# zynthbox/libzl

Hardware: AMD Instinct MI355X
Metric: voice-samples/sec at 1024 voices x 256-frame blocks; % HBM roofline (higher is better)
Workload: dtype f32

## Files before the change

libzl_amd/build.py:

```python
from __future__ import annotations

import os
import shutil
import subprocess
import sys

ROOT = os.path.dirname(os.path.dirname(os.path.abspath(__file__)))
CSRC = os.path.join(ROOT, "libzl_amd", "csrc")
LIBDIR = os.path.join(ROOT, "libzl_amd", "lib")
LIB = os.path.join(LIBDIR, "libzlhip.so")

HIP_SOURCES = ["zl_kernels.hip", "zl_stretch.hip", "zl_overview.hip", "zl_onset.hip", "zl_tempo.hip", "zl_pitch.hip", "zl_loudness.hip", "zl_loop.hip", "zl_key.hip", "zl_xfade.hip", "zl_decode.hip", "zl_resample.hip", "zl_engine.cpp", "zl_clip_calls.cpp", "zl_libzl.cpp", "zl_group.cpp"]
HEADERS = ["zl_types.h", "zl_arena.h", "zl_plan.h", "zl_order.h", "zl_pair.h", "zl_launch.h", "zl_render.h", "zl_kernels.h", "zl_host.h", "zl_sched.h", "zl_handoff.h", "zl_stretch.h", "zl_overview.h", "zl_onset.h", "zl_tempo.h", "zl_pitch.h", "zl_loudness.h", "zl_loop.h", "zl_key.h", "zl_xfade.h", "zl_decode.h", "zl_resample.h", "zl_group.h", "zl_member.h", "zl_owned.h", "zl_engine_impl.h",
           os.path.join("..", "..", "include", "zlhip.h"), os.path.join("..", "..", "include", "libzl_hotpath.h")]


def _hipcc() -> str:
    for cand in (os.environ.get("HIPCC"), shutil.which("hipcc"), "/opt/rocm/bin/hipcc"):
        if cand and os.path.exists(cand):
            return cand
    raise RuntimeError("hipcc not found (needed to build libzlhip.so for gfx950)")


def _stale(target: str, deps: list[str]) -> bool:
# ... 144 lines not shown
    if ref is None:
        return None
    odir = os.path.join(ROOT, "oracle")
    target = REF_LIB_CONTRACTED if contracted else REF_LIB
    voice = os.path.join(ref, "lib", "SamplerSynthVoice.cpp")
    driver = os.path.join(odir, "ref_driver.cpp")
    shim = os.path.join(odir, "ref_shim")
    deps = [voice, driver, os.path.join(odir, "zl_oracle.c"), os.path.join(odir, "zl_oracle.h"), os.path.abspath(__file__)]
    deps += [os.path.join(d, f) for d, _, fs in os.walk(shim) for f in fs]
    deps += [os.path.join(ref, "lib", f) for f in os.listdir(os.path.join(ref, "lib")) if f.endswith(".h")]
    if not force and not _stale(target, deps):
        return target
    os.makedirs(os.path.dirname(target), exist_ok=True)
    fp = ["-O2", "-mfma", "-ffp-contract=fast"] if contracted else ["-O2", "-ffp-contract=off", "-fno-fast-math"]
    cobj = os.path.join(os.path.dirname(target), "zl_oracle_fma.o" if contracted else "zl_oracle.o")
    cmds = [["gcc", "-std=c11", "-O2", "-ffp-contract=off", "-fno-fast-math", "-fPIC", "-c", os.path.join(odir, "zl_oracle.c"), "-o", cobj],
            ["g++", "-std=c++17"] + fp + ["-fPIC", "-shared", "-Wall", "-Wl,-Bsymbolic", "-I", shim, "-I", odir, "-I", os.path.join(ref, "lib"),
                                          "-o", target, voice, driver, cobj, "-lm", "-lpthread"]]
    for cmd in cmds:
        res = subprocess.run(cmd, capture_output=True, text=True)
        if res.returncode != 0:
            sys.stderr.write(res.stdout + res.stderr)
            raise RuntimeError("building the reference voice failed")
    return target


_ZLHIP_H = os.path.join(_INC, "zlhip.h")
_NO_CONTRACT = ["-ffp-contract=off", "-fno-fast-math"]


def _build_harness(name: str, source: str, headers: list, flags: list, force: bool = False) -> str:
    hdir = os.path.join(ROOT, "tests", "cpu_harness")
    target = os.path.join(hdir, "_build", f"lib{name}.so")
    src = os.path.join(hdir, source)
    if force or _stale(target, [src] + [os.path.join(CSRC, h) for h in headers]):
        os.makedirs(os.path.dirname(target), exist_ok=True)
        cmd = ["g++", "-std=c++17", "-O2"] + flags + ["-fPIC", "-shared", "-Wl,-Bsymbolic", "-I", CSRC, "-I", os.path.join(ROOT, "include"), "-o", target, src]
        res = subprocess.run(cmd, capture_output=True, text=True)
        if res.returncode != 0:
            sys.stderr.write(res.stdout + res.stderr)
            raise RuntimeError(f"building the CPU test harness {source} failed")
    return target


def build_cpu_harness(force: bool = False) -> str:
    target = _build_harness("zl_plan_host", "plan_host.cpp", ["zl_types.h", "zl_plan.h", "zl_render.h", "zl_host.h", _ZLHIP_H], _NO_CONTRACT, force)
    _build_harness("zl_sched_host", "sched_host.cpp", ["zl_sched.h", _ZLHIP_H], _NO_CONTRACT + ["-Wall"], force)
    _build_harness("zl_stretch_host", "stretch_host.cpp", ["zl_stretch.h", "zl_types.h"], _NO_CONTRACT + ["-Wall", "-pthread"], force)
    return target


def build_order_harness(force: bool = False) -> str:
    return _build_harness("zl_order_host", "order_host.cpp", ["zl_types.h", "zl_plan.h", "zl_order.h", "zl_host.h", _ZLHIP_H], _NO_CONTRACT + ["-Wall", "-Wno-unused-function"], force)


def build_order_summary_harness(force: bool = False) -> str:
    return _build_harness("zl_order_summary_host", "order_summary_host.cpp", ["zl_types.h", "zl_order.h"], ["-Wall", "-Wno-unused-function"], force)


def build_ongrid_harness(force: bool = False) -> str:
    return _build_harness("zl_ongrid_host", "ongrid_host.cpp", ["zl_types.h", "zl_render.h"], _NO_CONTRACT + ["-Wall", "-Wno-unused-function"], force)


def build_ongrid_pk_harness(force: bool = False) -> str:
    return _build_harness("zl_ongrid_pk_host", "ongrid_pk_host.cpp", ["zl_types.h", "zl_render.h"], _NO_CONTRACT + ["-Wall", "-Wno-unused-function"], force)


def build_pair_harness(force: bool = False) -> str:
    return _build_harness("zl_pair_host", "pair_host.cpp", ["zl_pair.h"], ["-Wall"], force)


def build_pair_wrap_harness(force: bool = False) -> str:
    plan_host = os.path.join("..", "..", "tests", "cpu_harness", "plan_host.cpp")
    return _build_harness("zl_pair_wrap_host", "pair_wrap_host.cpp", ["zl_types.h", "zl_plan.h", "zl_render.h", "zl_host.h", _ZLHIP_H, plan_host],
                          _NO_CONTRACT + ["-Wall", "-Wno-unused-function"], force)


def build_pair_scalar_harness(force: bool = False) -> str:
    plan_host = os.path.join("..", "..", "tests", "cpu_harness", "plan_host.cpp")
    return _build_harness("zl_pair_scalar_host", "pair_scalar_host.cpp", ["zl_types.h", "zl_plan.h", "zl_render.h", "zl_order.h", "zl_pair.h", "zl_host.h", _ZLHIP_H, plan_host],
                          _NO_CONTRACT + ["-Wall", "-Wno-unused-function"], force)


def build_group_harness(force: bool = False) -> str:
    return _build_harness("zl_group_host", "group_host.cpp", ["zl_types.h", "zl_plan.h", "zl_host.h", "zl_group.h", _ZLHIP_H], _NO_CONTRACT + ["-Wall", "-Wno-unused-function"], force)


def build_overview_harness(force: bool = False) -> str:
    return _build_harness("zl_overview_host", "overview_host.cpp", ["zl_types.h", "zl_overview.h"], ["-Wall"], force)


def build_onset_harness(force: bool = False) -> str:
    return _build_harness("zl_onset_host", "onset_host.cpp", ["zl_types.h", "zl_stretch.h", "zl_overview.h", "zl_onset.h"], _NO_CONTRACT + ["-Wall", "-pthread"], force)


def build_tempo_harness(force: bool = False) -> str:
    return _build_harness("zl_tempo_host", "tempo_host.cpp", ["zl_types.h", "zl_stretch.h", "zl_overview.h", "zl_onset.h", "zl_tempo.h"], _NO_CONTRACT + ["-Wall", "-pthread"], force)


def build_pitch_harness(force: bool = False) -> str:
    return _build_harness("zl_pitch_host", "pitch_host.cpp", ["zl_types.h", "zl_stretch.h", "zl_overview.h", "zl_onset.h", "zl_pitch.h"], _NO_CONTRACT + ["-Wall", "-pthread"], force)


def build_loudness_harness(force: bool = False) -> str:
    return _build_harness("zl_loudness_host", "loudness_host.cpp", ["zl_types.h", "zl_overview.h", "zl_loudness.h"], _NO_CONTRACT + ["-Wall", "-pthread"], force)


def build_loop_harness(force: bool = False) -> str:
    return _build_harness("zl_loop_host", "loop_host.cpp", ["zl_types.h", "zl_stretch.h", "zl_overview.h", "zl_onset.h", "zl_pitch.h", "zl_loop.h"], _NO_CONTRACT + ["-Wall", "-pthread"], force)


def build_key_harness(force: bool = False) -> str:
    return _build_harness("zl_key_host", "key_host.cpp", ["zl_types.h", "zl_stretch.h", "zl_overview.h", "zl_onset.h", "zl_pitch.h", "zl_key.h"], _NO_CONTRACT + ["-Wall", "-pthread"], force)


def build_xfade_harness(force: bool = False) -> str:
    return _build_harness("zl_xfade_host", "xfade_host.cpp", ["zl_types.h", "zl_stretch.h", "zl_overview.h", "zl_onset.h", "zl_pitch.h", "zl_xfade.h", _ZLHIP_H], _NO_CONTRACT + ["-Wall"], force)


def build_decode_harness(force: bool = False) -> str:
    return _build_harness("zl_decode_host", "decode_host.cpp", ["zl_types.h", "zl_decode.h"], _NO_CONTRACT + ["-Wall"], force)


def build_resample_harness(force: bool = False) -> str:
    return _build_harness("zl_resample_host", "resample_host.cpp", ["zl_types.h", "zl_resample.h"], _NO_CONTRACT + ["-Wall"], force)


def build_arena_harness(force: bool = False) -> str:
    return _build_harness("zl_arena_host", "arena_host.cpp", ["zl_types.h", "zl_stretch.h", "zl_arena.h"], ["-Wall"], force)


def build_launch_harness(force: bool = False) -> str:
    return _build_harness("zl_launch_host", "launch_host.cpp", ["zl_types.h", "zl_order.h", "zl_pair.h", "zl_launch.h"], ["-Wall", "-Wno-unused-function"], force)


if __name__ == "__main__":
    force = "--force" in sys.argv
    print(build_engine(force=force, verbose=True))
    print(build_oracle(force=force))
```

libzl_amd/csrc/zl_engine.cpp:

```cpp
#include <hip/hip_runtime.h>
#include <sys/resource.h>

#include <algorithm>
#include <atomic>
#include <cmath>
#include <cstdio>
#include <cstdlib>
#include <chrono>
#include <cstring>
#include <mutex>
#include <string>
#include <utility>
#include <vector>

#include "../../include/zlhip.h"
#include "zl_engine_impl.h"
#include "zl_kernels.h"
#include "zl_member.h"
#include "zl_order.h"
#include "zl_pair.h"
#include "zl_plan.h"
#include "zl_render.h"

#define ZL_RT_SPLIT_MIN_VOICES 32
// ... 713 lines not shown
                              const zlhip_passthrough_params *fan_params, float *fan_out_dev, void *stream)
{
    return render_batch_impl(e, nblocks, nframes, clocks, bus_out_dev, 0, 0, fan_params, fan_out_dev, stream);
}

static int render_batch_impl(zlhip_engine *e, int32_t nblocks, int32_t nframes, const zlhip_clock *clocks, float *bus_out_dev, long long bus_stride,
                             long long ch_stride, const zlhip_passthrough_params *fan_params, float *fan_out_dev, void *stream)
{
    if (!e || !clocks || ((fan_params == nullptr) != (fan_out_dev == nullptr))) return ZLHIP_ERR_INVALID;
    if (nblocks < 1 || nblocks > e->cfg.max_batch_blocks) return fail(e, ZLHIP_ERR_CAPACITY, "nblocks exceeds max_batch_blocks");
    if (nframes < 1 || nframes > e->cfg.max_frames)
        return fail(e, ZLHIP_ERR_INVALID, "nframes must be in [1, max_frames]");
    if (e->failed) return fail(e, ZLHIP_ERR_STATE, "engine failed (the resident kernel stopped answering in the middle of a cycle): destroy it");
    ZL_HIP(e, hipSetDevice(e->device));
    { int r_ = rt_stop(e); if (r_ != ZLHIP_OK) return r_; }
    hipStream_t s = stream ? (hipStream_t)stream : e->stream;

    static const bool callStamps = std::getenv("ZL_CALL_STAMPS") != nullptr;
    const auto tEnter = std::chrono::steady_clock::now();
    zlhip_engine::CallSlot &c = e->slots[e->callIndex & 1u];
    if (c.inflight) {
        ZL_HIP(e, hipEventSynchronize(c.done));
        c.inflight = false;
        int hrc = harvest_slot(e, c);
        if (hrc != ZLHIP_OK) return hrc;
    }
    c.doneGen ^= 1u; c.done = c.doneEv[c.doneGen];
    const auto tSlot = std::chrono::steady_clock::now();
    bool regular = true;
    for (int k = 0; k < nblocks; ++k) {
        ZlHostControl::fill_clock(c.clocks.h[k], clocks[k], nframes);
        if (c.clocks.h[k].usecs_per_frame >= (1ull << 21) || c.clocks.h[k].usecs_per_frame != c.clocks.h[0].usecs_per_frame
            || (k > 0 && c.clocks.h[k].current_usecs < c.clocks.h[k - 1].current_usecs)) regular = false;
    }

    ZlBatch A; std::memset(&A, 0, sizeof A);
    A.V = e->V; A.B = e->cfg.num_buses; A.VPB = e->cfg.voices_per_bus; A.N = nframes; A.Ktot = nblocks;
    A.G = pick_group(e, nblocks, nframes);
    A.groups = (A.VPB + A.G - 1) / A.G;
    A.NB = zl_k2_narrow_buses(nblocks, A.groups, A.VPB, A.B, nframes);
    A.clocks_regular = regular ? 1 : 0;
    A.mode = e->cfg.mode;
    A.ongrid = zl_ongrid_switch();
    A.staged = (e->staged && !e->trace && nframes % 64 == 0) ? 1 : 0;
    A.sounds = e->dSounds; A.clips = e->dClips; A.arena = e->arena;
    A.voices = e->dVoices; A.reports = c.dReports; A.pass_cache = e->dPassCache;
    A.bus = bus_out_dev ? bus_out_dev : e->dBus; A.stats = c.dStats;
    A.bus_stride = bus_stride; A.ch_stride = ch_stride;
    A.trace = 0; A.pos_trace = nullptr;
    int32_t *traceBase = nullptr;
    if (e->trace) {
        const size_t need = (size_t)nblocks * e->V * nframes;
        if (need > e->traceInts) {
            ZlQuiesce quiet(e);
            e->traceInts = 0;
            ZL_HIP(e, e->dTrace.alloc(need));
            e->traceInts = need;
        }
        ZL_HIP(e, hipMemsetAsync(e->dTrace, 0xff, need * sizeof(int32_t), s));
        A.trace = 1; traceBase = e->dTrace; e->traceK = nblocks; e->traceN = nframes;
#ifdef ZL_STAMPS
        A.trace = 0;
#endif
    }

    static const int windowMulEnv = [] { const char *v = std::getenv("ZL_WINDOW_MUL"); const int m = v ? std::atoi(v) : 0; return m < 0 ? 0 : (m > 64 ? 64 : m); }();
    bool cheap = nframes >= 256;
    for (const ZlHostVoice &hv : e->hc.voices) if (hv.isPlaying && !hv.cheapPlan) { cheap = false; break; }
    int windowMul = windowMulEnv;
    if (windowMul == 0) windowMul = cheap ? 4 : 1;
    const size_t mul = e->maxGroups > 1 ? 1 : (size_t)windowMul;
    std::vector<std::pair<int, int>> &wins = e->wins;
    zlhip_engine::CallSlot &prev = e->slots[(e->callIndex + 1u) & 1u];
    const bool behindPrev = prev.inflight && hipEventQuery(prev.done) == hipErrorNotReady;
    const char *fw = std::getenv("ZL_FIRST_WINDOW_FRAMES");
    const int fwFrames = fw ? std::atoi(fw) : 0;
    zl_plan_windows(nblocks, nframes, e->windowBlocks, e->windowFrames, e->windowCap, mul, e->ps[1].hdr != nullptr, behindPrev, fw ? &fwFrames : nullptr, wins);
    const int nwin = (int)wins.size();
    const int phaseMode = [] { const char *v = std::getenv("ZL_K2_PHASE_ORDER"); return v ? std::atoi(v) : 1; }();
    const double loopFrames = phaseMode == 1 ? e->hc.phase_order_loop_frames() : INFINITY;
    const int pairMode = [] { const char *v = std::getenv("ZL_K2_PAIR"); return v ? std::atoi(v) : 1; }();
    const int stageNorun = [] { const char *v = std::getenv("ZL_K2_STAGE_NORUN"); return v ? (std::atoi(v) != 0 ? 1 : 0) : 1; }();
    const int pairScalar = [] { const char *v = std::getenv("ZL_K2_PAIR_SCALAR"); return v ? (std::atoi(v) != 0 ? 1 : 0) : 1; }();
    const bool direct = e->bnc.sink.on && e->bnc.sink.hostDev && A.groups == 1;
    const ZlK2Switches &k2sw = zl_k2_switches();
    auto k2Launch = [&](int K, bool orderTable) {
        ZlK2In in;
        in.mode = A.mode; in.N = nframes; in.K = K; in.B = A.B; in.groups = A.groups; in.NB = A.NB;
        in.staged = A.staged; in.trace = A.trace; in.ongrid = A.ongrid; in.fan = fan_out_dev != nullptr; in.host_out = direct;
        in.order_mode = phaseMode; in.call_blocks = nblocks; in.bounce = e->bnc.sink.on; in.order_table = orderTable; in.loop_frames = loopFrames;
        in.pair_mode = pairMode; in.cheap = cheap;
        return zl_k2_launch(in, k2sw);
    };
    {
        size_t need = 0;
        for (const auto &wk : wins) { const ZlK2Launch L = k2Launch(wk.second, true); if (L.order) need = std::max(need, zl_order_ints((int)L.gz, wk.second, e->V)); }
        if (need > e->ps[0].orderInts || (e->ps[1].hdr != nullptr && need > e->ps[1].orderInts)) {
            ZlQuiesce quiet(e);
            for (auto &q : e->ps) {
                if (need <= q.orderInts || q.hdr == nullptr) continue;
                q.orderInts = 0;
                ZL_HIP(e, q.order.alloc(need));
                q.orderInts = need;
            }
        }
    }
    const bool overlap = e->ps[1].hdr != nullptr && (nwin > 1 || behindPrev || e->bnc.active);
    hipStream_t ps = overlap ? e->planStream : s;
    if (e->lastPlanStream && e->lastPlanStream != ps && e->lastPlanEvent) ZL_HIP(e, hipStreamWaitEvent(ps, e->lastPlanEvent, 0));
    if (nblocks == 1) { A.inline_clock = 1; A.clock0 = c.clocks.h[0]; A.fuse_assemble = 1; }
    if (fan_out_dev) {
        for (int b = 0; b < A.B; ++b) c.pass.h[b] = pass_params(fan_params[b]);
        ZL_HIP(e, hipMemcpyAsync(c.dPass, c.pass.h, (size_t)A.B * sizeof(ZlPassParams), hipMemcpyHostToDevice, ps));
        A.pass = c.dPass; A.fan = fan_out_dev;
    }
    int rc = upload_ops(e, c, A);
    if (rc != ZLHIP_OK) return rc;
    if (e->profiling) {
        if (behindPrev && prev.profiled && e->lastRenderStream == s) c.beginEv = prev.done;
        else { ZL_HIP(e, hipEventRecord(c.evBegin, s)); c.beginEv = c.evBegin; }
    }
    e->lastRenderStream = s;
    const unsigned phase = e->ps[1].hdr != nullptr ? e->setPhase : 0u;
    const bool fusedReports = k2Launch(wins[0].second, false).scans_levels && !(e->bnc.sink.on && !direct);
    c.fusedDone = fusedReports;
    for (int w = 0; w < nwin; ++w) {
        zlhip_engine::PlanSet &q = e->ps[(phase + (unsigned)w) & 1u];
        ZlBatch Aw = A;
        Aw.k0 = wins[(size_t)w].first;
        Aw.K = wins[(size_t)w].second;
        Aw.clocks = c.clocks.d + Aw.k0;
        Aw.levels = e->dLevels + (size_t)Aw.k0 * A.B;
        Aw.pos_trace = traceBase ? traceBase + (size_t)Aw.k0 * e->V * nframes : nullptr;
        Aw.vconst = q.vconst; Aw.runs = q.runs; Aw.tsegs = q.tsegs; Aw.plan_hdr = q.hdr; Aw.plan_seg0 = q.seg0; Aw.plan_seg1 = q.seg1;
        Aw.ctl_P = q.ctlP; Aw.ctl_env = q.ctlEnv; Aw.partials = q.partials;
        Aw.ctl_next = q.ctlNext; Aw.sim_const = q.simConst;
        Aw.ctl_slots = e->ctlSlotsOverride >= 0 ? std::min<int>(e->ctlSlotsOverride, (int)(e->ctlPoolFrames / (size_t)nframes)) : (int)std::min<size_t>(e->ctlPoolFrames / (size_t)nframes, 0x7fffffff);
        Aw.ctl_base = q.ctlBase;
        q.ctlBase += (unsigned long long)Aw.K * (unsigned long long)e->V + 1ull;
        const ZlK2Launch L = k2Launch(Aw.K, q.order != nullptr);
        Aw.order = L.order ? q.order : nullptr;
        if (zl_pair_scalar_window(pairScalar, L.kernel == ZL_K2_PAIR_PHASE_RENDER, L.order, q.pairTab != nullptr && Aw.K <= e->windowCap, A.VPB)) {
            Aw.ongrid |= ZL_ONGRID_SCALAR;
            zl_batch_set_pair_tab(Aw, q.pairTab);
        }
        if (w > 0) { Aw.n_op_ranges = 0; Aw.ops = nullptr; Aw.op_ranges = nullptr; Aw.n_clip_edits = 0; Aw.clip_edits = nullptr; }
        if (ps != s && q.used) ZL_HIP(e, hipStreamWaitEvent(ps, q.renderedEv, 0));
        ZL_KERNEL(e, zl_launch_apply_ops(Aw, ps));
        ZL_KERNEL(e, zl_launch_plan(Aw, e->forceSlow, ps));
        if (ps != s && e->asmStream && !Aw.fuse_assemble) {
            ZL_HIP(e, hipEventRecord(q.k1done, ps));
            ZL_HIP(e, hipStreamWaitEvent(e->asmStream, q.k1done, 0));
            ZL_KERNEL(e, zl_launch_assemble(Aw, e->asmStream));
            if (L.order) ZL_KERNEL(e, zl_launch_order(Aw, q.order, (int)L.gz, stageNorun, e->asmStream));
            ZL_HIP(e, hipEventRecord(q.planned, e->asmStream));
            ZL_HIP(e, hipStreamWaitEvent(s, q.planned, 0));
        } else {
            if (!Aw.fuse_assemble) ZL_KERNEL(e, zl_launch_assemble(Aw, ps));
            if (L.order) ZL_KERNEL(e, zl_launch_order(Aw, q.order, (int)L.gz, stageNorun, ps));
            if (ps != s) {
                ZL_HIP(e, hipEventRecord(q.planned, ps));
                ZL_HIP(e, hipStreamWaitEvent(s, q.planned, 0));
            }
        }
        const bool k3 = !L.scans_levels;
        if (direct) { Aw.host_out = e->bnc.sink.hostDev; Aw.host_fmt = e->bnc.sink.pcm ? 1 : 0; Aw.host_total = (long long)e->bnc.sink.totalFrames; Aw.host_k0 = 0; }
        const bool closes = fusedReports && w == nwin - 1;
        if (fusedReports) { Aw.fused_reports = 1; Aw.rep_gain = e->dGain; Aw.rep_host = c.reports.d; Aw.rep_host_gain = c.gain.d; Aw.rep_host_stats = c.stats.d; }
        Aw.pair = (L.kernel == ZL_K2_PAIR_RENDER || L.kernel == ZL_K2_PAIR_PHASE_RENDER) ? 1 : 0;
        hipEvent_t k2stop = closes ? c.done : (e->profiling ? c.evK2[2 * (size_t)w + 1] : nullptr);
        ZL_KERNEL(e, zl_launch_render(Aw, L, s, e->profiling ? c.evK2[2 * (size_t)w] : nullptr, k2stop));
        if (k3) ZL_KERNEL(e, zl_launch_finalize(Aw, nullptr, s));
        if (e->bnc.sink.on && !direct) { int d_ = bounce_deliver_window(e, A.bus, 0, Aw.B, Aw.k0, Aw.K, nblocks, nframes, s); if (d_ != ZLHIP_OK) return d_; }
        if (e->ps[1].hdr != nullptr) {
            if (k2stop && !k3) q.renderedEv = k2stop;
            else { ZL_HIP(e, hipEventRecord(q.rendered, s)); q.renderedEv = q.rendered; }
            q.used = true;
        }
    }
    c.windows = nwin;
    if (ps != s) { ZL_HIP(e, hipEventRecord(e->evPlanTail, ps)); e->lastPlanEvent = e->evPlanTail; }
    else e->lastPlanEvent = c.done;
    e->lastPlanStream = ps;
    if (e->ps[1].hdr != nullptr) e->setPhase = (phase + (unsigned)nwin) & 1u;
    if (fusedReports) {
        if (e->profiling) c.profiled = true;
    } else {
        ZL_KERNEL(e, zl_launch_reports(c.dReports, e->V, e->dGain, c.reports.d, c.gain.d, c.dStats, c.stats.d, s, e->profiling ? nullptr : c.done));
        if (e->profiling) { ZL_HIP(e, hipEventRecord(c.evEnd, s)); c.profiled = true; ZL_HIP(e, hipEventRecord(c.done, s)); }
    }
    c.inflight = true;
    if (s != e->stream) e->joins[0] = c.done;
    e->latest = &c;
    e->callIndex += 1;
    e->lastK = nblocks; e->lastN = nframes; e->lastBus = bus_stride ? nullptr : A.bus; e->lastWindows = nwin;
    e->outstanding = true; e->reportsFresh = true;
    if (callStamps) {
        const auto tEnd = std::chrono::steady_clock::now();
        auto us = [](auto a, auto b) { return std::chrono::duration<double, std::micro>(b - a).count(); };
        std::fprintf(stderr, "zlhip_render_batch #%u: slot wait %.0f us, commands %.0f us, %d window(s)\n", e->callIndex - 1, us(tEnter, tSlot), us(tSlot, tEnd), nwin);
    }
    return ZLHIP_OK;
}

int zlhip_host_alloc(size_t bytes, void **out)
{
    if (!out || bytes == 0) return ZLHIP_ERR_INVALID;
    *out = nullptr;
    return hipHostMalloc(out, bytes) == hipSuccess ? ZLHIP_OK : ZLHIP_ERR_CAPACITY;
}

void zlhip_host_free(void *p) { if (p) { ZlQuiesce quiet(nullptr); (void)hipHostFree(p); } }

static int bounce_body(zlhip_engine *e, int64_t nblocks, int32_t nframes, const zlhip_clock *clocks, void *host_out, bool pcm, int64_t chunk)
{
    constexpr int NBUF = zlhip_engine::Bounce::NBUF;
    zlhip_engine::Bounce &q = e->bnc;
    const size_t total = (size_t)nblocks * (size_t)nframes;
    static const bool stamps = std::getenv("ZL_BOUNCE_STAMPS") != nullptr;
    auto now_us = [] { return std::chrono::duration<double, std::micro>(std::chrono::steady_clock::now().time_since_epoch()).count(); };
    const double t00 = stamps ? now_us() : 0.0;
    const int directMode = [] { const char *v = std::getenv("ZL_BOUNCE_DIRECT"); return v ? std::atoi(v) : 2; }();
    void *hostDev = nullptr;
    if (directMode >= (pcm ? 1 : 2)) {
        if (hipHostGetDevicePointer(&hostDev, host_out, 0) != hipSuccess) { hostDev = nullptr; (void)hipGetLastError(); }
    }
// ... 638 lines not shown
```

libzl_amd/csrc/zl_kernels.hip:

```cpp
#include <hip/hip_runtime.h>
#include <hip/hip_ext.h>
#include <algorithm>
#include <cstddef>
#include "zl_types.h"
#include "zl_plan.h"
#include "zl_render.h"
#include "zl_order.h"
#include "zl_pair.h"
#include "zl_kernels.h"

static __device__ __forceinline__ void zl_apply_clip_edit(const ZlBatch &A, const ZlClipEdit *ed, int lane)
{
    static_assert(offsetof(ZlClip, slice_pos) == ZL_CLIP_HEAD_BYTES && sizeof(ZlClip) % 16 == 0 && offsetof(ZlClipEdit, c) % 16 == 0, "clip record layout");
    const int clip = ed->clip;
    const int n16 = ed->full ? (int)(sizeof(ZlClip) / 16) : ZL_CLIP_HEAD_BYTES / 16;
    const uint4 *src = reinterpret_cast<const uint4 *>(&ed->c);
    uint4 *dst = reinterpret_cast<uint4 *>(const_cast<ZlClip *>(A.clips) + clip);
    for (int w = lane; w < n16; w += 64) dst[w] = src[w];
}

__global__ void zl_k0_apply_ops(const ZlBatch A)
{
    const int opGroups = (A.n_op_ranges + 63) / 64;
    if ((int)blockIdx.x >= opGroups) {
// ... 1470 lines not shown

template <uint32_t MODE, int BPW, bool ST>
__global__ void __launch_bounds__(256, ST ? 3 : (MODE & (ZL_MODE_HERMITE | ZL_MODE_FIX_DELAY)) == 0 ? (BPW == 1 ? ZL_K2_WAVES_LINEAR : 5)
                                              : ((MODE & ZL_MODE_HERMITE) == 0 && BPW == 1) ? ZL_K2_WAVES_LINEAR : ZL_K2_MINWAVES) zl_k2_render(const ZlBatch A)
{
    zl_k2_body<MODE, BPW, ST>(A, blockIdx.x, blockIdx.y, blockIdx.z, gridDim.x, gridDim.y);
}

template <uint32_t MODE>
__global__ void __launch_bounds__(256, (MODE & ZL_MODE_HERMITE) == 0 ? ZL_K2_WAVES_LINEAR : ZL_K2_MINWAVES) zl_k2_phase_render(const ZlBatch A)
{
    zl_k2_body<MODE, 1, false, true, true>(A, blockIdx.x, blockIdx.y, blockIdx.z, gridDim.x, gridDim.y);
}

#ifndef ZL_K2_PAIR_WAVES
#define ZL_K2_PAIR_WAVES 4
#endif
#define ZL_K2_PAIR_LDS 18432

typedef uint64_t zl_u64x8 __attribute__((ext_vector_type(8)));
typedef float zl_f16 __attribute__((ext_vector_type(16)));
#define ZL_CONST_AS __attribute__((address_space(4)))
static __device__ __forceinline__ zl_f2 zl_pk_pan_s(zl_f2 pan, zl_f2 ms)
{
    zl_f2 r; asm("v_pk_mul_f32 %0, %1, %2 op_sel:[0,0] op_sel_hi:[1,0]" : "=v"(r) : "s"(pan), "v"(ms)); return r;
}
template <int SEL>
static __device__ __forceinline__ void zl_mix_acc_ongrid_pk_s(zl_f2 &acc, zl_f2 x, zl_f2 pan)
{
    zl_f2 ms = SEL == 0 ? zl_pk_sumdiff(x) : SEL == 1 ? zl_pk_sumdiff_lo(x) : zl_pk_sumdiff_hi(x);
    ms.x = 0.5f * ms.x;
    acc = zl_pk_add(acc, zl_pk_side(zl_pk_pan_s(pan, ms), ms));
}
template <bool MONO>
static __device__ __forceinline__ void zl_k2_pair_fast(const uint64_t *addr, const uint64_t *pan, int nch, int f0,
                                                       float &accL0, float &accR0, float &accL1, float &accR1)
{
    constexpr int U = 8;
    const ZL_CONST_AS zl_u64x8 *at = reinterpret_cast<const ZL_CONST_AS zl_u64x8 *>(reinterpret_cast<uintptr_t>(addr));
    const ZL_CONST_AS zl_f16 *pt = reinterpret_cast<const ZL_CONST_AS zl_f16 *>(reinterpret_cast<uintptr_t>(pan));
    zl_f2 acc0 = {accL0, accR0}, acc1 = {accL1, accR1};
    zl_u64x8 a = at[0];
    for (int c = 0; c < nch; ++c) {
        zl_f4a8 d4[MONO ? 1 : U];
        zl_f2   d2[MONO ? U : 1];
        const uint32_t ob = zl_k2_ongrid_offset((uint32_t)f0 << (MONO ? 2 : 3));
#pragma unroll
        for (int u = 0; u < U; ++u) {
            if (MONO) d2[u] = zl_k2_ongrid_load<zl_f2a4b>(a[u], ob);
            else      d4[u] = zl_k2_ongrid_load<zl_f4a8>(a[u], ob);
        }
        const zl_f16 p = pt[c];
        a = at[c + 1 < nch ? c + 1 : c];
        __builtin_amdgcn_sched_barrier(0);
#pragma unroll
        for (int u = 0; u < U; ++u) {
            const zl_f2 pu = {p[2 * u], p[2 * u + 1]};
            if (MONO) {
                zl_mix_acc_ongrid_pk_s<1>(acc0, d2[u], pu);
                zl_mix_acc_ongrid_pk_s<2>(acc1, d2[u], pu);
            } else {
                zl_mix_acc_ongrid_pk_s<0>(acc0, __builtin_shufflevector(d4[u], d4[u], 0, 1), pu);
                zl_mix_acc_ongrid_pk_s<0>(acc1, __builtin_shufflevector(d4[u], d4[u], 2, 3), pu);
            }
        }
    }
    accL0 = acc0.x; accR0 = acc0.y; accL1 = acc1.x; accR1 = acc1.y;
}
static __device__ __forceinline__ int zl_k2_pair_fast_kind(const uint64_t *tab, int K, int V, int k, int v0, int v1)
{
    const ZL_CONST_AS uint32_t *bw = reinterpret_cast<const ZL_CONST_AS uint32_t *>(reinterpret_cast<uintptr_t>(tab + zl_pair_tab_fast(K, V)));
    const int G = (V + 63) / 64;
    bool all = true, anyMono = false, allMono = true;
    for (int g = v0 >> 6; g <= (v1 - 1) >> 6; ++g) {
        const size_t i = (size_t)k * (size_t)G + (size_t)g;
        const uint32_t w = (bw[i >> 1] >> ((i & 1) * 16)) & 0xffffu;
        const uint32_t need = zl_pair_group_need(v0, v1, g);
        all = all && (w & need) == need;
        anyMono = anyMono || ((w >> 8) & need) != 0u;
        allMono = allMono && ((w >> 8) & need) == need;
    }
    return !all ? 0 : allMono ? 2 : anyMono ? 0 : 1;
}
template <bool ORD>
static __device__ __forceinline__ void zl_k2_pair_body(const ZlBatch &A)
{
    constexpr uint32_t MODE = 0;
    constexpr int U = ZL_K2_U, UP = ZL_K2_U_PAIR, UW = ZL_K2_U_PAIR_WRAP, CH = ZL_K2_CHUNK;
    static_assert(UP == U || 2 * UP == U, "the pair chunk walks a chunk class of U voices whole or in halves");
    static_assert(UW == U || 2 * UW == U, "and so does the chunk with loop restarts");
    __shared__ ZlBlockPlan  s_plan[CH];
    __shared__ ZlVoiceConst s_vc[CH];
    __shared__ int s_cls[CH];
    __shared__ int s_chunk[CH / U];
    __shared__ ZlUnit s_unit[CH];
    __shared__ int   s_pk[2][4];
    __shared__ float s_sq[2][4];

    const int N = A.N, V = A.V;
    const int f0 = 2 * (int)threadIdx.x;
    const unsigned by = blockIdx.y, bz = blockIdx.z;
    const int ky = (int)gridDim.y, xq = ky >> 3, xr = ky & 7, xx = (int)(by & 7u);
    const int ys = xx * xq + (xx < xr ? xx : xr) + (int)(by >> 3);
    const int k = ORD ? A.order[(size_t)bz * A.K + ys] : ys;
    __builtin_assume(k >= 0 && k < 65536);
    const int bus = (int)bz;
    const int v0 = bus * A.VPB, vlim = (bus + 1) * A.VPB;
    const int v1 = (v0 + A.G < vlim) ? v0 + A.G : vlim;
    const bool wantPeak = __builtin_amdgcn_readfirstlane((int)(A.k0 + k == A.Ktot - 1)) != 0;
    const int32_t *dead_tail = ORD ? A.order + zl_order_tail_dead((int)gridDim.z, A.K, 0) : nullptr;
    const bool norun = ORD && __builtin_amdgcn_readfirstlane((int)(k >= A.order[zl_order_tail_run_end((int)gridDim.z, A.K, (int)bz)])) != 0;

    float accL0 = 0.0f, accR0 = 0.0f, accL1 = 0.0f, accR1 = 0.0f;
    int fastKind = 0;
    if (ORD && (A.ongrid & ZL_ONGRID_SCALAR) && norun && !wantPeak)
        fastKind = zl_k2_pair_fast_kind(zl_batch_pair_tab(A), A.K, V, __builtin_amdgcn_readfirstlane(k), v0, v1);
    if (fastKind != 0) {
        const uint64_t *addr = zl_batch_pair_tab(A) + (size_t)__builtin_amdgcn_readfirstlane(k) * (size_t)V + (size_t)v0;
        const uint64_t *pan = zl_batch_pair_tab(A) + zl_pair_tab_pan(A.K, V) + (size_t)v0;
        if (fastKind == 2) zl_k2_pair_fast<true>(addr, pan, (v1 - v0) >> 3, f0, accL0, accR0, accL1, accR1);
        else               zl_k2_pair_fast<false>(addr, pan, (v1 - v0) >> 3, f0, accL0, accR0, accL1, accR1);
    } else
    for (int vb = v0; vb < v1; vb += CH) {
        const int nv = (v1 - vb < CH) ? v1 - vb : CH;
        if (vb != v0) __syncthreads();
        for (int i = threadIdx.x; i < CH; i += blockDim.x) {
            ZlVoiceConst vc;
            ZlBlockPlan pl;
            if (norun) zl_k2_stage_load<false>(A, k, vb, i, nv, vc, pl, dead_tail);
            else       zl_k2_stage_load<true>(A, k, vb, i, nv, vc, pl, nullptr);
            const int cls = zl_k2_stage_class<MODE>(A, vc, pl);
            s_unit[i] = zl_k2_stage_unit<MODE>(A, vc, pl, cls);
            s_vc[i] = vc;
            s_plan[i] = pl;
            s_cls[i] = cls;
            zl_k2_stage_chunks<U>(cls, i, s_chunk);
        }
        __syncthreads();
        for (int c0 = 0; c0 < nv; c0 += U) {
            const int cc = __builtin_amdgcn_readfirstlane(s_chunk[c0 / U]);
            if (cc == 0) {
            } else if ((cc & 132) == 132) {
#pragma unroll
                for (int h = 0; h < U; h += UP) {
                    if (wantPeak) {
                        if (cc & 16) zl_k2_chunk_ongrid_pair<true, UP, true>(A, s_vc, s_unit, c0 + h, vb, f0, accL0, accR0, accL1, accR1);
                        else         zl_k2_chunk_ongrid_pair<false, UP, true>(A, s_vc, s_unit, c0 + h, vb, f0, accL0, accR0, accL1, accR1);
                    }
                    else if (cc & 16) zl_k2_chunk_ongrid_pair<true, UP, false>(A, s_vc, s_unit, c0 + h, vb, f0, accL0, accR0, accL1, accR1);
                    else              zl_k2_chunk_ongrid_pair<false, UP, false>(A, s_vc, s_unit, c0 + h, vb, f0, accL0, accR0, accL1, accR1);
                }
            } else if ((cc & 256) && !wantPeak) {
#pragma unroll
                for (int h = 0; h < U; h += UW) {
                    if (cc & 16) zl_k2_chunk_ongrid_pair_wrap<true, UW>(A, s_plan, s_vc, s_unit, c0 + h, f0, accL0, accR0, accL1, accR1);
                    else         zl_k2_chunk_ongrid_pair_wrap<false, UW>(A, s_plan, s_vc, s_unit, c0 + h, f0, accL0, accR0, accL1, accR1);
                }
            } else {
#pragma nounroll
                for (int h = 0; h < 2; ++h) {
                    const int fc = f0 + h;
                    const double fd = (double)fc;
                    float accL = h ? accL1 : accL0, accR = h ? accR1 : accR0;
                    if ((cc & 124) == 100)      zl_k2_chunk_simple<MODE, false, true, true, U>(A, s_plan, s_vc, s_unit, c0, vb, fc, fd, wantPeak, accL, accR);
                    else if ((cc & 92) == 68)   zl_k2_chunk_simple<MODE, false, false, true, U>(A, s_plan, s_vc, s_unit, c0, vb, fc, fd, wantPeak, accL, accR);
                    else if ((cc & 28) == 4)    zl_k2_chunk_simple<MODE, false, false, false, U>(A, s_plan, s_vc, s_unit, c0, vb, fc, fd, wantPeak, accL, accR);
                    else if ((cc & 20) == 4)    zl_k2_chunk_simple<MODE, true, false, false, U>(A, s_plan, s_vc, s_unit, c0, vb, fc, fd, wantPeak, accL, accR);
                    else if ((cc & 124) == 116) zl_k2_chunk_simple_mono<MODE, false, true, true, U>(A, s_plan, s_vc, s_unit, c0, vb, fc, fd, wantPeak, accL, accR);
                    else if ((cc & 92) == 84)   zl_k2_chunk_simple_mono<MODE, false, false, true, U>(A, s_plan, s_vc, s_unit, c0, vb, fc, fd, wantPeak, accL, accR);
                    else if ((cc & 28) == 20)   zl_k2_chunk_simple_mono<MODE, false, false, false, U>(A, s_plan, s_vc, s_unit, c0, vb, fc, fd, wantPeak, accL, accR);
                    else if ((cc & 20) == 20)   zl_k2_chunk_simple_mono<MODE, true, false, false, U>(A, s_plan, s_vc, s_unit, c0, vb, fc, fd, wantPeak, accL, accR);
                    else {
                        constexpr int H = U / 2;
                        const size_t pbase = (size_t)k * V + vb;
                        for (int q = 0; q < U; q += H) {
                            if (cc & 2) zl_k2_chunk<MODE, true, H>(A, s_plan, s_vc, s_cls, c0 + q, pbase, vb, fc, wantPeak, accL, accR);
                            else        zl_k2_chunk<MODE, false, H>(A, s_plan, s_vc, s_cls, c0 + q, pbase, vb, fc, wantPeak, accL, accR);
                        }
                    }
                    if (h) { accL1 = accL; accR1 = accR; } else { accL0 = accL; accR0 = accR; }
                }
            }
        }
    }

    {
        const long long KN = (long long)A.Ktot * N;
        float *outL = A.bus + (long long)bus * (A.bus_stride ? A.bus_stride : 2 * KN) + (long long)(A.k0 + k) * N;
        float *outR = outL + (A.ch_stride ? A.ch_stride : KN);
        const bool written1 = f0 + 2 < N;
        outL[f0 + 1] = accL0; outR[f0 + 1] = accR0;
        if (written1) { outL[f0 + 2] = accL1; outR[f0 + 2] = accR1; }
        if (f0 == 0)  { outL[0] = 0.0f; outR[0] = 0.0f; }
        if (A.levels) {
            const float bL = written1 ? accL1 : 0.0f, bR = written1 ? accR1 : 0.0f;
            const int pa = zl_sample_to_peak_int(accL0), pb = zl_sample_to_peak_int(bL), pc = zl_sample_to_peak_int(accR0), pd = zl_sample_to_peak_int(bR);
            int pkL[2], pkR[2]; float sqL[2], sqR[2];
            zl_wave_levels4_pair(pb > pa ? pb : pa, pd > pc ? pd : pc, accL0 * accL0 + bL * bL, accR0 * accR0 + bR * bR, pkL, pkR, sqL, sqR);
            const int w = (int)(threadIdx.x >> 6) * 2;
            if ((threadIdx.x & 63) == 0) {
                s_pk[0][w] = pkL[0]; s_pk[1][w] = pkR[0]; s_sq[0][w] = sqL[0]; s_sq[1][w] = sqR[0];
                s_pk[0][w + 1] = pkL[1]; s_pk[1][w + 1] = pkR[1]; s_sq[0][w + 1] = sqL[1]; s_sq[1][w + 1] = sqR[1];
            }
            __syncthreads();
            if (threadIdx.x == 0) {
                ZlBlockLevels lv; lv.peak_l = 0; lv.peak_r = 0; lv.sumsq_l = 0.0f; lv.sumsq_r = 0.0f;
                for (int t = 0; t < 4; ++t) {
                    lv.peak_l = s_pk[0][t] > lv.peak_l ? s_pk[0][t] : lv.peak_l;
                    lv.peak_r = s_pk[1][t] > lv.peak_r ? s_pk[1][t] : lv.peak_r;
                    lv.sumsq_l += s_sq[0][t]; lv.sumsq_r += s_sq[1][t];
                }
                A.levels[(size_t)k * A.B + bus] = lv;
            }
        }
    }

    if (A.fused_reports && A.k0 + k == A.Ktot - 1) {
        __syncthreads();
        for (int v = v0 + (int)threadIdx.x; v < v1; v += (int)blockDim.x) {
            const uint4 *src = reinterpret_cast<const uint4 *>(&A.reports[v]);
            uint4 a = src[0];
            const uint4 b = src[1];
            a.z = __hip_atomic_load(&A.reports[v].peak_bits, __ATOMIC_RELAXED, __HIP_MEMORY_SCOPE_AGENT);
            const float gn = __uint_as_float(a.z) * 0.5f;
            A.rep_gain[v] = gn;
            if (A.rep_host) { uint4 *dst = reinterpret_cast<uint4 *>(&A.rep_host[v]); dst[0] = a; dst[1] = b; A.rep_host_gain[v] = gn; }
        }
        if (bus == 0 && threadIdx.x == 0 && A.rep_host_stats) {
            const unsigned long long sb = A.stats->source_bytes, sl = A.stats->slow_blocks, af = A.stats->active_frames;
            A.rep_host_stats->source_bytes = sb; A.rep_host_stats->slow_blocks = sl; A.rep_host_stats->active_frames = af;
            A.stats->source_bytes = 0; A.stats->slow_blocks = 0; A.stats->active_frames = 0;
        }
    }
}

__global__ void __launch_bounds__(128, ZL_K2_PAIR_WAVES) zl_k2_pair_render(const ZlBatch A) { zl_k2_pair_body<false>(A); }
__global__ void __launch_bounds__(128, ZL_K2_PAIR_WAVES) zl_k2_pair_phase_render(const ZlBatch A) { zl_k2_pair_body<true>(A); }

static __device__ __forceinline__ void zl_k3_body(const ZlBatch &A, const float *bus_in, int k, int bus);
template <uint32_t MODE, bool WIDE>
__global__ void __launch_bounds__(256) __attribute__((amdgpu_waves_per_eu(2, 2))) zl_k_rt_loop(const ZlBatch A0, ZlRtShared *sh, ZlRtDev *dev, unsigned long long first_seq, unsigned long long idle_ticks,
                                                    float *gain_out, ZlReport *host_reports, float *host_gain, ZlOpRange *dev_ranges, int vw)
{
    __shared__ unsigned long long s_cmd[ZL_RT_CMD_WORDS + 1];
    __shared__ int s_go, s_last;
    __shared__ ZlClock s_clk0;
    __shared__ ZlPassParams s_pass;
    __shared__ uint32_t s_pass_seq;
    const int tid = threadIdx.x, lane = tid & 63;
    if (tid == 0) s_pass_seq = 0u;
    const int z = blockIdx.x, W = gridDim.x;
    const int vbeg = WIDE ? z * vw : z * A0.VPB, vend = WIDE ? vbeg + vw : vbeg + A0.VPB;
    unsigned long long last = first_seq;
    if (z == 0 && tid == 0) __hip_atomic_store(&sh->state, 1u, __ATOMIC_RELAXED, __HIP_MEMORY_SCOPE_SYSTEM);
    for (;;) {
        if (tid == 0) {
            int go = 0;
            if (z == 0) {
                const unsigned long long t0 = __builtin_amdgcn_s_memrealtime();
                for (;;) {
                    const unsigned long long q = __hip_atomic_load(&sh->cmd_seq, __ATOMIC_RELAXED, __HIP_MEMORY_SCOPE_SYSTEM);
                    if (q != last) {
                        if (!WIDE) __hip_atomic_store(&dev->pub_seq, q, __ATOMIC_RELAXED, __HIP_MEMORY_SCOPE_AGENT);
                        s_cmd[0] = q; go = 1;
                        break;
// ... 652 lines not shown
```

libzl_amd/csrc/zl_pair.h:

```cpp
#pragma once
#include <stdint.h>

inline bool zl_pair_shape(uint32_t mode, int N, int K, int NB, int groups, int staged, int trace, bool fan, bool host_out, int ongrid)
{
    return mode == 0u && N == 256 && K > 1 && NB == 1 && groups == 1 && !staged && !trace && !fan && !host_out && ongrid != 0;
}

inline bool zl_pair_window(int sw, bool shape, bool cheap)
{
    if (sw == 2) return shape;
    return sw == 1 && shape && cheap;
}

inline bool zl_pair_scalar_window(int sw, bool pair, bool phase_order, bool have_tab, int VPB)
{
    return sw != 0 && pair && phase_order && have_tab && VPB > 0 && (VPB % 8) == 0;
}
```

libzl_amd/csrc/zl_render.h:

```cpp
#pragma once
#include "zl_types.h"
#include <math.h>
#include <stddef.h>
#include <string.h>

ZL_HD inline void zl_eval_control(const ZlBlockPlan &pl, int f, double &P, float &env)
{
    const bool seg1 = f >= pl.n1;
    const int n0 = seg1 ? pl.n1 : 0;
    P = fma((double)(f - n0), seg1 ? pl.step1 : pl.step, seg1 ? pl.P1 : pl.P0);
    env = (float)fma((double)(f - n0), (double)(seg1 ? pl.estep1 : pl.estep0), (double)(seg1 ? pl.E1 : pl.env));
}

struct ZlHermiteW { float w0, w1, w2, w3; };
ZL_HD inline ZlHermiteW zl_hermite_weights(float a)
{
    ZlHermiteW w;
    const float t = a * a;
    w.w0 = fmaf(fmaf(-0.5f, a, 1.0f), a, -0.5f) * a;
    w.w1 = fmaf(fmaf(1.5f, a, -2.5f), t, 1.0f);
    w.w2 = fmaf(fmaf(-1.5f, a, 2.0f), a, 0.5f) * a;
    w.w3 = fmaf(0.5f, a, -0.5f) * t;
    return w;
}
// ... 36 lines not shown
    if (!inb) l = 0.0f;
    if (!(stereo && inb)) r = l;
    const float mSignal = 0.5f * (l + r);
    const float sSignal = l - r;
    lout = lpan * mSignal + sSignal;
    rout = rpan * mSignal - sSignal;
}

ZL_HD inline bool zl_voice_ongrid(uint32_t mode, int enabled, bool simple, bool unit, bool interior, double P0, double step, int sound_flags)
{
    return enabled != 0 && simple && unit && interior && step == 1.0 && P0 == (double)(int)P0 && (sound_flags & ZL_SOUND_FINITE) != 0
        && (mode & (ZL_MODE_HERMITE | ZL_MODE_FIX_GAIN)) == 0;
}

#define ZL_ONGRID_ON   1
#define ZL_ONGRID_WRAP 2
ZL_HD inline bool zl_voice_ongrid2(uint32_t mode, int ongrid, int sound_flags, int cls, int n_active, int plan_flags, bool gains_finite,
                                   int nseg, int n1, int N, double step, double step1, double P0, double P1, int sample_duration)
{
    return (ongrid & ZL_ONGRID_ON) != 0 && (ongrid & ZL_ONGRID_WRAP) != 0 && (mode & (ZL_MODE_HERMITE | ZL_MODE_FIX_GAIN)) == 0
        && (sound_flags & ZL_SOUND_FINITE) != 0
        && cls == 1 && n_active == N && (plan_flags & ZL_PLAN_ENV) == 0 && gains_finite
        && nseg == 2 && n1 > 0 && n1 < N
        && step == 1.0 && step1 == 1.0
        && P0 >= 0.0 && P0 < 1073741824.0 && P0 == (double)(int)P0 && P1 >= 0.0 && P1 < 1073741824.0 && P1 == (double)(int)P1
        && P0 + (double)(n1 - 1) < (double)sample_duration && P1 + (double)(N - 1 - n1) < (double)sample_duration;
}

struct ZlWrapLane { int x, y; bool straddle; };
ZL_HD inline ZlWrapLane zl_ongrid2_lane(int ipos, int alt, int n1, int f0)
{
    ZlWrapLane w;
    w.x = (f0 >= n1 ? alt : ipos) + f0;
    w.straddle = f0 + 1 == n1;
    w.y = w.straddle ? alt + f0 + 1 : w.x;
    return w;
}

ZL_HD inline int zl_voice_block_class(uint32_t mode, int ongrid, int trace, int N, const ZlVoiceConst &vc, const ZlBlockPlan &pl)
{
    int cls = (pl.flags & ZL_PLAN_ACTIVE) ? (1 | ((pl.flags & ZL_PLAN_SLOW) ? 2 : 0)) : 0;
    const float gprod = vc.lgain * vc.rgain * vc.clip_volume * pl.env;
    if (cls == 1 && pl.nseg <= 2 && !(pl.flags & ZL_PLAN_ENV) && pl.n_active == N && (vc.channels == 1 || vc.channels == 2) && !trace
        && (gprod - gprod) == 0.0f && (uint32_t)vc.sample_duration < 0x1ffffff0u)
    {
        const bool HM = (mode & ZL_MODE_HERMITE) != 0;
        const double Pmax = fma((double)(N - 1), pl.step, pl.P0);
        const bool interior = pl.nseg == 1 && pl.P0 >= (HM ? 1.0 : 0.0) && Pmax < (double)(vc.sample_duration - (HM ? 1 : 0));
        cls |= 4 | (pl.nseg == 2 ? 8 : 0) | (vc.channels == 1 ? 16 : 0) | ((pl.nseg == 1 && pl.step == 1.0 && pl.P0 < 1073741824.0) ? 32 : 0)
             | (interior ? 64 : 0);
        cls |= zl_voice_ongrid(mode, ongrid, true, (cls & 32) != 0, interior, pl.P0, pl.step, vc.pad[0]) ? 128 : 0;
        cls |= zl_voice_ongrid2(mode, ongrid, vc.pad[0], cls & 3, pl.n_active, pl.flags, true, pl.nseg, pl.n1, N, pl.step, pl.step1, pl.P0, pl.P1,
                                vc.sample_duration) ? 256 : 0;
    }
    return cls;
}

#define ZL_ONGRID_SCALAR 4
ZL_HD inline size_t zl_pair_tab_pan(int K, int V) { return (size_t)K * (size_t)V; }
ZL_HD inline size_t zl_pair_tab_fast(int K, int V) { return (size_t)K * (size_t)V + (size_t)V; }
ZL_HD inline size_t zl_pair_tab_words(int K, int V) { return zl_pair_tab_fast(K, V) + ((size_t)K * (size_t)((V + 63) / 64) * 2 + 7) / 8; }
ZL_HD inline bool zl_voice_block_fast(int cls) { return (cls & (4 | 64 | 128)) == (4 | 64 | 128); }
ZL_HD inline uint64_t zl_ongrid_addr0(uint64_t arena, uint64_t src_offset, double P0, bool mono)
{
    return arena + (src_offset << 2) + ((uint64_t)(uint32_t)(int)P0 << (mono ? 2 : 3));
}
ZL_HD inline uint32_t zl_pair_fast_bits(unsigned long long fast, unsigned long long mono)
{
    uint32_t w = 0;
    for (int c = 0; c < 8; ++c) {
        const unsigned f = (unsigned)(fast >> (8 * c)) & 255u, m = (unsigned)(mono >> (8 * c)) & 255u;
        if (f == 255u && (m == 0u || m == 255u)) w |= 1u << c;
        if (m == 255u) w |= 256u << c;
    }
    return w;
}
ZL_HD inline uint32_t zl_pair_group_need(int v0, int v1, int g)
{
    const int lo = v0 > 64 * g ? v0 : 64 * g, hi = v1 < 64 * g + 64 ? v1 : 64 * g + 64;
    if (hi <= lo) return 0u;
    return ((1u << ((hi - lo) >> 3)) - 1u) << ((lo - 64 * g) >> 3);
}

ZL_HD inline void zl_mix_frame_ongrid(float x0l, float x0r, float lpan, float rpan, float &lout, float &rout)
{
    const float mSignal = 0.5f * (x0l + x0r);
    const float sSignal = x0l - x0r;
    lout = lpan * mSignal + sSignal;
    rout = rpan * mSignal - sSignal;
}

ZL_HD inline void zl_mix_frame_ongrid_pk(float x0l, float x0r, float lpan, float rpan, float &lout, float &rout)
{
    const float sum = x0l + x0r, dif = x0l + (-x0r);
    const float m = sum * 0.5f, s = dif * 1.0f;
    const float lm = lpan * m, rm = rpan * m;
    lout = lm + s;
    rout = rm + (-s);
}

ZL_HD inline bool zl_f32_bits_finite(uint32_t bits) { return (bits & 0x7f800000u) != 0x7f800000u; }
inline bool zl_all_finite(const float *x, size_t n)
{
    uint32_t worst = 0;
    for (size_t i = 0; i < n; ++i) { uint32_t b; memcpy(&b, x + i, sizeof b); worst |= zl_f32_bits_finite(b) ? 0u : 1u; }
    return worst == 0;
}

ZL_HD inline void zl_pass_pan(const ZlPassParams &p, float &lm, float &rm)
{
    const float a = 1 - p.pan, b = 1 + p.pan;
    lm = (1.0f < a) ? 1.0f : a;
    rm = (1.0f < b) ? 1.0f : b;
}
ZL_HD inline void zl_pass_pair(const ZlPassParams &p, float amount, float lm, float rm, float sl, float sr, float &ol, float &orr)
{
    if (p.muted)                            { ol = 0.0f; orr = 0.0f; }
    else if (p.pan == 0 && amount == 0)     { ol = 0.0f; orr = 0.0f; }
    else if (p.pan == 0 && amount == 1)     { ol = sl;   orr = sr; }
    else                                    { ol = amount * sl * lm; orr = amount * sr * rm; }
}

template <uint32_t MODE>
ZL_HD inline void zl_render_frame(const ZlVoiceConst &vc, const float *src, double P, float env,
                                  float &lout, float &rout, int &pos_out)
{
    int pos; float alpha;
    zl_split_position(P, pos, alpha);
    const bool inb = vc.sample_duration > pos && pos >= 0;
    const bool stereo = vc.channels > 1;
    const bool wide = (MODE & ZL_MODE_HERMITE) && inb && (pos - 1 >= 0) && (pos + 2 <= vc.sample_duration);
    const int p = inb ? pos : 0;
    ZlTaps t;
    t.xml = t.xmr = t.x2l = t.x2r = 0.0f;
    if (stereo) {
        t.x0l = src[2 * p]; t.x0r = src[2 * p + 1]; t.x1l = src[2 * p + 2]; t.x1r = src[2 * p + 3];
        if (wide) { t.xml = src[2 * p - 2]; t.xmr = src[2 * p - 1]; t.x2l = src[2 * p + 4]; t.x2r = src[2 * p + 5]; }
    } else {
        t.x0l = src[p]; t.x1l = src[p + 1]; t.x0r = 0.0f; t.x1r = 0.0f;
        if (wide) { t.xml = src[p - 1]; t.x2l = src[p + 2]; }
    }
    zl_mix_frame<MODE>(t, alpha, inb, wide, stereo, vc.lgain, vc.rgain, env, vc.clip_volume, vc.lpan, vc.rpan, lout, rout);
    pos_out = pos;
}

ZL_HD inline int16_t zl_pcm16(float x)
{
    const double d = (double)x;
    int32_t q;
    if (d <= -1.0) q = INT32_MIN;
    else if (d >= 1.0) q = INT32_MAX;
    else if (d != d) q = 0;
    else q = (int32_t)rint(2147483647.0 * d);
    return (int16_t)(q >> 16);
}
```

Baseline: 2356 billion.

## Mix scalar fast-path chunks with staged chunks per pass in pair render

Before, the scalar fast path ran only when every voice chunk in the block qualified. Now per-chunk fast and mono bits are read for each 128-voice pass. Runs of fast chunks go through the scalar record path and the remaining chunks are staged and rendered normally, skipping staging loads for the fast chunks. This lets partially eligible blocks avoid most staging work, at the cost of extra mask reads and run-splitting control flow. A pass whose fast chunks mix mono and non-mono falls back to full staging.

Result: no change. 2352 billion (median of 2 runs) (-0.2%).

```diff
diff --git a/libzl_amd/build.py b/libzl_amd/build.py
--- a/libzl_amd/build.py
+++ b/libzl_amd/build.py
@@ -250,6 +250,13 @@
                           _NO_CONTRACT + ["-Wall", "-Wno-unused-function"], force)
 
 
+def build_pair_mixed_harness(force: bool = False) -> str:
+    hdir = os.path.join("..", "..", "tests", "cpu_harness")
+    return _build_harness("zl_pair_mixed_host", "pair_mixed_host.cpp", ["zl_types.h", "zl_plan.h", "zl_render.h", "zl_order.h", "zl_pair.h", "zl_host.h", _ZLHIP_H,
+                                                                         os.path.join(hdir, "plan_host.cpp"), os.path.join(hdir, "pair_scalar_host.cpp")],
+                          _NO_CONTRACT + ["-Wall", "-Wno-unused-function"], force)
+
+
 def build_group_harness(force: bool = False) -> str:
     return _build_harness("zl_group_host", "group_host.cpp", ["zl_types.h", "zl_plan.h", "zl_host.h", "zl_group.h", _ZLHIP_H], _NO_CONTRACT + ["-Wall", "-Wno-unused-function"], force)
 
diff --git a/libzl_amd/csrc/zl_engine.cpp b/libzl_amd/csrc/zl_engine.cpp
--- a/libzl_amd/csrc/zl_engine.cpp
+++ b/libzl_amd/csrc/zl_engine.cpp
@@ -819,6 +819,7 @@
     const int pairMode = [] { const char *v = std::getenv("ZL_K2_PAIR"); return v ? std::atoi(v) : 1; }();
     const int stageNorun = [] { const char *v = std::getenv("ZL_K2_STAGE_NORUN"); return v ? (std::atoi(v) != 0 ? 1 : 0) : 1; }();
     const int pairScalar = [] { const char *v = std::getenv("ZL_K2_PAIR_SCALAR"); return v ? (std::atoi(v) != 0 ? 1 : 0) : 1; }();
+    const int pairMixed = [] { const char *v = std::getenv("ZL_K2_PAIR_MIXED"); return v ? (std::atoi(v) != 0 ? 1 : 0) : 1; }();
     const bool direct = e->bnc.sink.on && e->bnc.sink.hostDev && A.groups == 1;
     const ZlK2Switches &k2sw = zl_k2_switches();
     auto k2Launch = [&](int K, bool orderTable) {
@@ -878,7 +879,7 @@
         const ZlK2Launch L = k2Launch(Aw.K, q.order != nullptr);
         Aw.order = L.order ? q.order : nullptr;
         if (zl_pair_scalar_window(pairScalar, L.kernel == ZL_K2_PAIR_PHASE_RENDER, L.order, q.pairTab != nullptr && Aw.K <= e->windowCap, A.VPB)) {
-            Aw.ongrid |= ZL_ONGRID_SCALAR;
+            Aw.ongrid |= ZL_ONGRID_SCALAR | (zl_pair_mixed_window(pairMixed, true) ? ZL_ONGRID_MIXED : 0);
             zl_batch_set_pair_tab(Aw, q.pairTab);
         }
         if (w > 0) { Aw.n_op_ranges = 0; Aw.ops = nullptr; Aw.op_ranges = nullptr; Aw.n_clip_edits = 0; Aw.clip_edits = nullptr; }
diff --git a/libzl_amd/csrc/zl_kernels.hip b/libzl_amd/csrc/zl_kernels.hip
--- a/libzl_amd/csrc/zl_kernels.hip
+++ b/libzl_amd/csrc/zl_kernels.hip
@@ -1576,6 +1576,18 @@
     }
     return !all ? 0 : allMono ? 2 : anyMono ? 0 : 1;
 }
+static __device__ __forceinline__ void zl_k2_pair_masks(const uint64_t *tab, int K, int V, int k, int vb, int v1, int nch, uint32_t &fmask, uint32_t &mmask)
+{
+    const ZL_CONST_AS uint32_t *bw = reinterpret_cast<const ZL_CONST_AS uint32_t *>(reinterpret_cast<uintptr_t>(tab + zl_pair_tab_fast(K, V)));
+    const int G = (V + 63) / 64, g0 = vb >> 6, glast = (v1 - 1) >> 6;
+    uint32_t w[3];
+#pragma unroll
+    for (int j = 0; j < 3; ++j) {
+        const size_t i = (size_t)k * (size_t)G + (size_t)(g0 + j);
+        w[j] = g0 + j <= glast ? (bw[i >> 1] >> ((i & 1) * 16)) & 0xffffu : 0u;
+    }
+    zl_pair_pass_masks(w[0], w[1], w[2], vb, nch, fmask, mmask);
+}
 template <bool ORD>
 static __device__ __forceinline__ void zl_k2_pair_body(const ZlBatch &A)
 {
@@ -1583,6 +1595,7 @@
     constexpr int U = ZL_K2_U, UP = ZL_K2_U_PAIR, UW = ZL_K2_U_PAIR_WRAP, CH = ZL_K2_CHUNK;
     static_assert(UP == U || 2 * UP == U, "the pair chunk walks a chunk class of U voices whole or in halves");
     static_assert(UW == U || 2 * UW == U, "and so does the chunk with loop restarts");
+    static_assert(U == 8 && CH == 16 * U, "the scalar records hold one bit per chunk of 8 voices; a pass's masks are 16 bits");
     __shared__ ZlBlockPlan  s_plan[CH];
     __shared__ ZlVoiceConst s_vc[CH];
     __shared__ int s_cls[CH];
@@ -1606,32 +1619,46 @@
     const bool norun = ORD && __builtin_amdgcn_readfirstlane((int)(k >= A.order[zl_order_tail_run_end((int)gridDim.z, A.K, (int)bz)])) != 0;
 
     float accL0 = 0.0f, accR0 = 0.0f, accL1 = 0.0f, accR1 = 0.0f;
+    const bool scalarOK = ORD && (A.ongrid & ZL_ONGRID_SCALAR) && norun && !wantPeak;
+    const bool mixedOK = scalarOK && (A.ongrid & ZL_ONGRID_MIXED) != 0;
+    const int ks = __builtin_amdgcn_readfirstlane(k);
     int fastKind = 0;
-    if (ORD && (A.ongrid & ZL_ONGRID_SCALAR) && norun && !wantPeak)
-        fastKind = zl_k2_pair_fast_kind(zl_batch_pair_tab(A), A.K, V, __builtin_amdgcn_readfirstlane(k), v0, v1);
-    if (fastKind != 0) {
-        const uint64_t *addr = zl_batch_pair_tab(A) + (size_t)__builtin_amdgcn_readfirstlane(k) * (size_t)V + (size_t)v0;
-        const uint64_t *pan = zl_batch_pair_tab(A) + zl_pair_tab_pan(A.K, V) + (size_t)v0;
-        if (fastKind == 2) zl_k2_pair_fast<true>(addr, pan, (v1 - v0) >> 3, f0, accL0, accR0, accL1, accR1);
-        else               zl_k2_pair_fast<false>(addr, pan, (v1 - v0) >> 3, f0, accL0, accR0, accL1, accR1);
-    } else
+    if (scalarOK && !mixedOK) fastKind = zl_k2_pair_fast_kind(zl_batch_pair_tab(A), A.K, V, ks, v0, v1);
     for (int vb = v0; vb < v1; vb += CH) {
         const int nv = (v1 - vb < CH) ? v1 - vb : CH;
-        if (vb != v0) __syncthreads();
-        for (int i = threadIdx.x; i < CH; i += blockDim.x) {
-            ZlVoiceConst vc;
-            ZlBlockPlan pl;
-            if (norun) zl_k2_stage_load<false>(A, k, vb, i, nv, vc, pl, dead_tail);
-            else       zl_k2_stage_load<true>(A, k, vb, i, nv, vc, pl, nullptr);
-            const int cls = zl_k2_stage_class<MODE>(A, vc, pl);
-            s_unit[i] = zl_k2_stage_unit<MODE>(A, vc, pl, cls);
-            s_vc[i] = vc;
-            s_plan[i] = pl;
-            s_cls[i] = cls;
-            zl_k2_stage_chunks<U>(cls, i, s_chunk);
-        }
-        __syncthreads();
-        for (int c0 = 0; c0 < nv; c0 += U) {
+        const int nch = (nv + U - 1) / U;
+        uint32_t fmask = 0u, mmask = 0u;
+        if (mixedOK) zl_k2_pair_masks(zl_batch_pair_tab(A), A.K, V, ks, vb, v1, nch, fmask, mmask);
+        else if (fastKind != 0) { fmask = (1u << nch) - 1u; mmask = fastKind == 2 ? fmask : 0u; }
+        const int kind = ORD ? zl_pair_pass_kind(fmask, mmask, nch) : ZL_PAIR_STAGED;
+        if (kind == ZL_PAIR_STAGED) fmask = 0u;
+        if (kind != ZL_PAIR_ALLFAST) {
+            if (vb != v0) __syncthreads();
+            for (int i = threadIdx.x; i < CH; i += blockDim.x) {
+                ZlVoiceConst vc;
+                ZlBlockPlan pl;
+                const int nvs = (ORD && ((fmask >> (i >> 3)) & 1u)) ? 0 : nv;
+                if (norun) zl_k2_stage_load<false>(A, k, vb, i, nvs, vc, pl, dead_tail);
+                else       zl_k2_stage_load<true>(A, k, vb, i, nvs, vc, pl, nullptr);
+                const int cls = zl_k2_stage_class<MODE>(A, vc, pl);
+                s_unit[i] = zl_k2_stage_unit<MODE>(A, vc, pl, cls);
+                s_vc[i] = vc;
+                s_plan[i] = pl;
+                s_cls[i] = cls;
+                zl_k2_stage_chunks<U>(cls, i, s_chunk);
+            }
+            __syncthreads();
+        }
+        for (int c = 0; c < nch; ) {
+          bool fast = false;
+          const int len = ORD ? zl_pair_next_run(fmask, c, nch, fast) : nch;
+          if (ORD && fast) {
+            const uint64_t *addr = zl_batch_pair_tab(A) + (size_t)ks * (size_t)V + (size_t)(vb + U * c);
+            const uint64_t *pan = zl_batch_pair_tab(A) + zl_pair_tab_pan(A.K, V) + (size_t)(vb + U * c);
+            if (mmask & fmask) zl_k2_pair_fast<true>(addr, pan, len, f0, accL0, accR0, accL1, accR1);
+            else               zl_k2_pair_fast<false>(addr, pan, len, f0, accL0, accR0, accL1, accR1);
+          } else
+          for (int c0 = U * c; c0 < U * (c + len); c0 += U) {
             const int cc = __builtin_amdgcn_readfirstlane(s_chunk[c0 / U]);
             if (cc == 0) {
             } else if ((cc & 132) == 132) {
@@ -1675,6 +1702,8 @@
                     if (h) { accL1 = accL; accR1 = accR; } else { accL0 = accL; accR0 = accR; }
                 }
             }
+          }
+          c = ORD ? __builtin_amdgcn_readfirstlane(c + len) : c + len;
         }
     }
 
diff --git a/libzl_amd/csrc/zl_pair.h b/libzl_amd/csrc/zl_pair.h
--- a/libzl_amd/csrc/zl_pair.h
+++ b/libzl_amd/csrc/zl_pair.h
@@ -16,3 +16,5 @@
 {
     return sw != 0 && pair && phase_order && have_tab && VPB > 0 && (VPB % 8) == 0;
 }
+
+inline bool zl_pair_mixed_window(int sw, bool scalar_window) { return sw != 0 && scalar_window; }
diff --git a/libzl_amd/csrc/zl_render.h b/libzl_amd/csrc/zl_render.h
--- a/libzl_amd/csrc/zl_render.h
+++ b/libzl_amd/csrc/zl_render.h
@@ -142,6 +142,29 @@
     return ((1u << ((hi - lo) >> 3)) - 1u) << ((lo - 64 * g) >> 3);
 }
 
+#define ZL_ONGRID_MIXED 8
+#define ZL_PAIR_STAGED  0
+#define ZL_PAIR_ALLFAST 1
+#define ZL_PAIR_MIXED   2
+ZL_HD inline void zl_pair_pass_masks(uint32_t w0, uint32_t w1, uint32_t w2, int vb, int nch, uint32_t &fmask, uint32_t &mmask)
+{
+    const int sh = (vb >> 3) & 7;
+    const uint32_t full = (1u << nch) - 1u;
+    fmask = (((w0 & 255u) | ((w1 & 255u) << 8) | ((w2 & 255u) << 16)) >> sh) & full;
+    mmask = ((((w0 >> 8) & 255u) | (((w1 >> 8) & 255u) << 8) | (((w2 >> 8) & 255u) << 16)) >> sh) & full;
+}
+ZL_HD inline int zl_pair_pass_kind(uint32_t fmask, uint32_t mmask, int nch)
+{
+    const uint32_t full = (1u << nch) - 1u, f = fmask & full, m = mmask & f;
+    if (f == 0u || (m != 0u && m != f)) return ZL_PAIR_STAGED;
+    return f == full ? ZL_PAIR_ALLFAST : ZL_PAIR_MIXED;
+}
+ZL_HD inline int zl_pair_next_run(uint32_t fmask, int c, int nch, bool &fast)
+{
+    fast = ((fmask >> c) & 1u) != 0u;
+    return __builtin_ctz(((fast ? ~fmask : fmask) >> c) | (1u << (nch - c)));
+}
+
 ZL_HD inline void zl_mix_frame_ongrid(float x0l, float x0r, float lpan, float rpan, float &lout, float &rout)
 {
     const float mSignal = 0.5f * (x0l + x0r);
```
